# Labbeti/conette-audio-captioning

Hardware: AMD Instinct MI355X
Metric: clips_per_sec (higher is better)
Workload: dtype bf16; 1 GPU; B=64/GPU x 10 s @ 32 kHz clips, ConvNeXt encoder + beam-3 KV-cached decode (min 3 / max 20 tokens, V=5631), synthetic seeded checkpoint; batch_per_gpu=64, global_batch=64, beam_size=3, parallelism=dp1, world_size_observed=1, allreduce_of_ones=1, decode_group=2, decode_streams=2, encode_streams=1, input_batches_rotated=4

## Files before the change

### conette-audio-captioning_amd/csrc/encoder.hip

```cpp
#include <stddef.h>

#include "ctx.h"
#include <type_traits>
#include <utility>

__device__ int g_cn_nonfinite;
__device__ __forceinline__ void cn_watch_stat(float v) {
  if (!(__builtin_fabsf(v) <= 3.0e38f)) atomicAdd(&g_cn_nonfinite, 1);
}

#include "gemm2.h"
#include "mlp_rc2.h"
#include "mlp_rs16.h"
#include "mlp_sp.h"
#include "down_fused.h"

template <typename XT>
__global__ __launch_bounds__(256) void cn_stem_mfma_kernel(const float* __restrict__ in, int F, int H0, long n_pos,
                                                           const float* __restrict__ w , const float* __restrict__ bias,
                                                           const float* __restrict__ ln_w, const float* __restrict__ ln_b,
                                                           XT* __restrict__ out) {
  __shared__ __attribute__((aligned(16))) float s_p[3 * 96];
  for (int i = threadIdx.x; i < 3 * 96; i += 256) s_p[i] = i < 96 ? bias[i] : i < 192 ? ln_w[i - 96] : ln_b[i - 192];
  const int lane = threadIdx.x & 63, j = lane & 31, h = lane >> 5;
  float a[3][8];
#pragma unroll
  for (int t = 0; t < 3; ++t)
#pragma unroll
    for (int s = 0; s < 8; ++s) a[t][s] = w[(4 * (s >> 1) + 2 * h + (s & 1)) * 96 + 32 * t + cn_rc2_chan(j)];
  __syncthreads();
  const long n_tiles = (n_pos + 31) >> 5;
  const long n_waves = (long)gridDim.x * 4;
  for (long tile = (long)blockIdx.x * 4 + (threadIdx.x >> 6); tile < n_tiles; tile += n_waves) {
    const long pos = tile * 32 + j;
    const long p = pos < n_pos ? pos : n_pos - 1;
    const int wq = (int)(p % 56);
    const long tt = p / 56;
    const int hh = (int)(tt % H0);
    const int b = (int)(tt / H0);
    f32x2 xv[4];
#pragma unroll
    for (int i = 0; i < 4; ++i) {
      const int r = 4 * hh - 4 + i;
      xv[i] = f32x2{0.f, 0.f};
      if (r >= 0 && r < F) xv[i] = *(const f32x2*)(in + ((size_t)b * F + r) * CN_N_MELS + 4 * wq + 2 * h);
    }
    f32x16 acc[3];
#pragma unroll
    for (int t = 0; t < 3; ++t)
#pragma unroll
      for (int u = 0; u < 2; ++u) {
        const f32x4 b0 = *(const f32x4*)(s_p + 32 * t + 16 * u + 8 * h), b1 = *(const f32x4*)(s_p + 32 * t + 16 * u + 8 * h + 4);
#pragma unroll
        for (int e = 0; e < 4; ++e) acc[t][8 * u + e] = b0[e], acc[t][8 * u + 4 + e] = b1[e];
      }
#pragma unroll
    for (int s = 0; s < 8; ++s)
#pragma unroll
      for (int t = 0; t < 3; ++t) acc[t] = __builtin_amdgcn_mfma_f32_32x32x2f32(a[t][s], xv[s >> 1][s & 1], acc[t], 0, 0, 0);
    float sum = 0.f;
#pragma unroll
    for (int t = 0; t < 3; ++t)
#pragma unroll
      for (int r = 0; r < 16; ++r) sum += acc[t][r];
    sum += __shfl_xor(sum, 32);
    const float mean = sum * (1.0f / 96.0f);
    float v2 = 0.f;
#pragma unroll
    for (int t = 0; t < 3; ++t)
#pragma unroll
      for (int r = 0; r < 16; ++r) {
        acc[t][r] -= mean;
        v2 = fmaf(acc[t][r], acc[t][r], v2);
      }
    v2 += __shfl_xor(v2, 32);
    const float rstd = 1.0f / sqrtf(v2 * (1.0f / 96.0f) + 1e-6f);
    if (pos < n_pos) {
      XT* o = out + (size_t)pos * 96 + 8 * h;
#pragma unroll
      for (int t = 0; t < 3; ++t)
#pragma unroll
        for (int u = 0; u < 2; ++u) {
          const int ch = 32 * t + 16 * u + 8 * h;
          float v[8];
#pragma unroll
          for (int q = 0; q < 2; ++q) {
            const f32x4 lw = *(const f32x4*)(s_p + 96 + ch + 4 * q), lb = *(const f32x4*)(s_p + 192 + ch + 4 * q);
#pragma unroll
            for (int e = 0; e < 4; ++e) v[4 * q + e] = acc[t][8 * u + 4 * q + e] * rstd * lw[e] + lb[e];
          }
          if constexpr (sizeof(XT) == 2) {
            *(cn_h8<XT>*)(o + 32 * t + 16 * u) = cn_h8<XT>{cn_from_f32<XT>(v[0]), cn_from_f32<XT>(v[1]), cn_from_f32<XT>(v[2]), cn_from_f32<XT>(v[3]),
                                                          cn_from_f32<XT>(v[4]), cn_from_f32<XT>(v[5]), cn_from_f32<XT>(v[6]), cn_from_f32<XT>(v[7])};
          } else {
            *(f32x4*)(o + 32 * t + 16 * u) = f32x4{v[0], v[1], v[2], v[3]};
            *(f32x4*)(o + 32 * t + 16 * u + 4) = f32x4{v[4], v[5], v[6], v[7]};
          }
        }
    }
  }
}

__device__ unsigned long long g_dw_prof[8];
#define DW_STAMP(i)                                                   \
  if (dbg) {                                                          \
    const unsigned long long t_ = clock64();                          \
    if ((threadIdx.x & 63) == 0) atomicAdd(&g_dw_prof[i], t_ - t_prev); \
    t_prev = t_;                                                      \
  }

template <int C, int S, int TH> struct DwTile {
  static constexpr int NCHUNK = C / 4;
  static constexpr int PITCH4 = NCHUNK | 1;
  static constexpr int PITCH = PITCH4 * 4;
};

template <int... U, typename F> __device__ __forceinline__ void cn_static_for(std::integer_sequence<int, U...>, F&& f) {
  (f(std::integral_constant<int, U>{}), ...);
}
__device__ __forceinline__ void cn_dw_pin1(float& v) { asm volatile("" : "+v"(v) : : "memory"); }
template <int TH, size_t... I> __device__ __forceinline__ void cn_dw_pin(float (&acc)[TH][4], std::index_sequence<I...>) {
  (cn_dw_pin1(acc[I / 4][I % 4]), ...);
}
__device__ __forceinline__ void cn_dw_opaque(unsigned& v) { asm volatile("" : "+v"(v)); }

template <typename T, typename XT, int C, int S, int TH, bool CLAMPED = false>
__global__ __launch_bounds__((C > 384 ? 384 : C) * S) void cn_dwconv_ln_kernel(const XT* __restrict__ x, int H, int W, int tiles_h,
                                                            int tiles_w, const float* __restrict__ dw_w ,
                                                            const unsigned* __restrict__ dw_wp ,
                                                            const float* __restrict__ dw_b,
                                                            const float* __restrict__ ln_w,
                                                            const float* __restrict__ ln_b, T* __restrict__ y,
                                                            int dbg) {
  extern __shared__ __attribute__((aligned(16))) char smem_raw[];
  float* s_v = (float*)smem_raw;
  unsigned long long t_prev = dbg ? clock64() : 0;
  constexpr int NP = TH * 4;
  constexpr int CT = C > 384 ? 384 : C;
  constexpr int PITCH = DwTile<C, S, TH>::PITCH;
  const int tid = threadIdx.x;
  const int c0 = tid % CT, sidx = tid / CT;
  int bid = cn_xcd_remap(blockIdx.x, gridDim.x);
  const int tw = bid % tiles_w;
  bid /= tiles_w;
  const int th = bid % tiles_h;
  const int b = bid / tiles_h;
  const int h0 = th * TH, w0 = tw * (4 * S) + sidx * 4;

  int wcl[10];
  bool wok[10];
#pragma unroll
  for (int q = 0; q < 10; ++q) {
    const int ww = w0 - 3 + q;
    wok[q] = (ww >= 0) && (ww < W);
    wcl[q] = min(max(ww, 0), W - 1) * C;
  }
#pragma unroll 1
  for (int c = c0; c < C; c += CT) {
  float acc[TH][4];
  const float bias = dw_b[c];
#pragma unroll
  for (int a = 0; a < TH; ++a)
#pragma unroll
    for (int e = 0; e < 4; ++e) acc[a][e] = bias;
  const XT* xb = x + (size_t)b * H * W * C + c;
  const bool interior = (h0 >= 3) && (h0 + TH + 3 <= H) && (w0 >= 3) && (w0 + 4 + 3 <= W);
  if constexpr (sizeof(XT) == 2) {
    static_assert(TH % 2 == 0, "row pairs");
    cn_h2 ke[3][7], ko[3][7];
#pragma unroll
    for (int a = 0; a < 3; ++a)
#pragma unroll
      for (int j = 0; j < 7; ++j) {
        ke[a][j] = __builtin_bit_cast(cn_h2, dw_wp[(a * 7 + j) * C + c]);
        ko[a][j] = __builtin_bit_cast(cn_h2, dw_wp[(21 + a * 7 + j) * C + c]);
      }
    DW_STAMP(0)
    auto fma_pair = [&](int r, const cn_h2 (&p)[10]) {
#pragma unroll
      for (int oh = 0; oh < TH; ++oh) {
        const int i = r - oh;
        if (i < -1 || i > 6) continue;
#pragma unroll
        for (int q = 0; q < 10; ++q)
#pragma unroll
          for (int ow = 0; ow < 4; ++ow) {
            const int j = q - ow;
            if (j < 0 || j > 6) continue;
            if (i == -1) acc[oh][ow] = fmaf((float)p[q][1], (float)ke[0][j][0], acc[oh][ow]);
            else if (i == 6) acc[oh][ow] = fmaf((float)p[q][0], (float)ko[2][j][1], acc[oh][ow]);
            else if ((i & 1) == 0) acc[oh][ow] = __builtin_amdgcn_fdot2(p[q], ke[i >> 1][j], acc[oh][ow], false);
            else acc[oh][ow] = __builtin_amdgcn_fdot2(p[q], ko[i >> 1][j], acc[oh][ow], false);
          }
      }
    };
    constexpr int NPR = (TH + 6) / 2;
    if constexpr (!CLAMPED) {
      const bool left = (w0 == 0), right = (w0 + 7 > W);
      const unsigned oL = 2u * (unsigned)((left ? 0 : w0 - 3) * C + c), oM = 2u * (unsigned)(w0 * C + c);
      const unsigned oR = 2u * (unsigned)((right ? w0 + 1 : w0 + 4) * C + c);
      constexpr unsigned SEL_PAIR = 0x05040100u, SEL_ZERO = 0x0c0c0c0cu;
      const unsigned selL = left ? SEL_ZERO : SEL_PAIR, selR = right ? SEL_ZERO : SEL_PAIR;
      const char* xc = (const char*)(x + (size_t)b * H * W * C);
      const bool rows_in = (h0 >= 3) && (h0 + TH + 3 <= H);
      const unsigned rows = ((1u << min(TH + 6, H + 3 - h0)) - 1u) & ~((1u << max(0, 3 - h0)) - 1u);
      auto conv = [&](auto check_rows) {
        constexpr bool CHECK = decltype(check_rows)::value;
        auto load_row = [&](int r, unsigned (&v)[10]) {
          const int hh = h0 - 3 + r;
          if (!CHECK || ((rows >> r) & 1u)) {
            const char* xr = xc + (size_t)hh * W * C * 2;
#pragma unroll
            for (int q = 0; q < 10; ++q)
              v[q] = *(const unsigned short*)(q < 3 ? xr + (size_t)oL + q * C * 2 : q < 7 ? xr + (size_t)oM + (q - 3) * C * 2 : xr + (size_t)oR + (q - 7) * C * 2);
          } else {
#pragma unroll
            for (int q = 0; q < 10; ++q) v[q] = 0u;
          }
        };
        auto pack = [&](const unsigned (&v0)[10], const unsigned (&v1)[10], cn_h2 (&p)[10]) {
#pragma unroll
          for (int q = 0; q < 10; ++q)
            p[q] = __builtin_bit_cast(cn_h2, __builtin_amdgcn_perm(v1[q], v0[q], q < 3 ? selL : q < 7 ? SEL_PAIR : selR));
        };
        auto pin = [&]() {
          if constexpr (CHECK) cn_dw_pin(acc, std::make_index_sequence<TH * 4>{});
        };
        unsigned a0[10], a1[10], b0[10], b1[10];
        cn_h2 p[10];
        load_row(0, a0);
        load_row(1, a1);
        cn_static_for(std::make_integer_sequence<int, (NPR + 1) / 2>{}, [&](auto k) {
          constexpr int u = 2 * decltype(k)::value;
          if (u + 1 < NPR) {
            load_row(2 * u + 2, b0);
            load_row(2 * u + 3, b1);
          }
          pack(a0, a1, p);
          fma_pair(2 * u, p);
          pin();
          if (u + 2 < NPR) {
            load_row(2 * u + 4, a0);
            load_row(2 * u + 5, a1);
          }
          if (u + 1 < NPR) {
            pack(b0, b1, p);
            fma_pair(2 * (u + 1), p);
            pin();
          }
        });
      };
      if (rows_in) conv(std::false_type{});
      else conv(std::true_type{});
    } else {
#pragma unroll
      for (int u = 0; u < NPR; ++u) {
        const int hh0 = h0 - 3 + 2 * u, hh1 = hh0 + 1;
        const bool ok0 = (hh0 >= 0) && (hh0 < H), ok1 = (hh1 >= 0) && (hh1 < H);
        const XT* x0 = xb + (size_t)min(max(hh0, 0), H - 1) * W * C;
        const XT* x1 = xb + (size_t)min(max(hh1, 0), H - 1) * W * C;
        XT v0[10], v1[10];
#pragma unroll
        for (int q = 0; q < 10; ++q) v0[q] = x0[wcl[q]], v1[q] = x1[wcl[q]];
        cn_h2 p[10];
#pragma unroll
        for (int q = 0; q < 10; ++q) p[q] = cn_h2{(ok0 && wok[q]) ? v0[q] : (XT)0.f, (ok1 && wok[q]) ? v1[q] : (XT)0.f};
        fma_pair(2 * u, p);
      }
    }
  } else {
  float k[49];
#pragma unroll
  for (int i = 0; i < 49; ++i) k[i] = dw_w[i * C + c];
  DW_STAMP(0)
  auto fma_row = [&](int r, const XT (&v)[10]) {
#pragma unroll
    for (int oh = 0; oh < TH; ++oh) {
      const int i = r - oh;
      if (i < 0 || i > 6) continue;
#pragma unroll
      for (int q = 0; q < 10; ++q)
#pragma unroll
        for (int ow = 0; ow < 4; ++ow) {
          const int j = q - ow;
          if (j < 0 || j > 6) continue;
          acc[oh][ow] = fmaf((float)v[q], k[i * 7 + j], acc[oh][ow]);
        }
    }
  };
  if (interior) {
    const XT* base = xb + ((size_t)(h0 - 3) * W + (w0 - 3)) * C;
    XT va[10], vb[10];
#pragma unroll
    for (int q = 0; q < 10; ++q) va[q] = base[q * C];
#pragma unroll
    for (int r = 0; r < TH + 6; r += 2) {
      if (r + 1 < TH + 6) {
        const XT* xr = base + (size_t)(r + 1) * W * C;
#pragma unroll
        for (int q = 0; q < 10; ++q) vb[q] = xr[q * C];
      }
      fma_row(r, va);
      if (r + 2 < TH + 6) {
        const XT* xr = base + (size_t)(r + 2) * W * C;
#pragma unroll
        for (int q = 0; q < 10; ++q) va[q] = xr[q * C];
      }
      if (r + 1 < TH + 6) fma_row(r + 1, vb);
    }
  } else {
#pragma unroll
    for (int r = 0; r < TH + 6; ++r) {
      const int hh = h0 - 3 + r;
      const bool hok = (hh >= 0) && (hh < H);
      const XT* xr = xb + (size_t)min(max(hh, 0), H - 1) * W * C;
      XT v[10];
#pragma unroll
      for (int q = 0; q < 10; ++q) v[q] = xr[wcl[q]];
#pragma unroll
      for (int q = 0; q < 10; ++q) v[q] = (hok && wok[q]) ? v[q] : (XT)0.f;
      fma_row(r, v);
    }
  }
  }
#pragma unroll
  for (int oh = 0; oh < TH; ++oh)
#pragma unroll
    for (int ow = 0; ow < 4; ++ow) s_v[((sidx * NP) + oh * 4 + ow) * PITCH + c] = acc[oh][ow];
  DW_STAMP(1)
  }
  __syncthreads();
  DW_STAMP(2)

  constexpr int NPOS = NP * S, NT = CT * S, PARTS = NT / NPOS, NCHUNK = C / 4, CPT = NCHUNK / PARTS;
  static_assert(NT % NPOS == 0 && NCHUNK % PARTS == 0, "LayerNorm thread mapping");
  float* s_ps = s_v + NPOS * PITCH;
  float* s_mean = s_ps + NPOS * PARTS;
  float* s_rstd = s_mean + NPOS;
  {
    const int pos = tid % NPOS, part = tid / NPOS;
    const float* row = s_v + pos * PITCH + part * 4;
    f32x4 seg[CPT];
    float sum = 0.f;
#pragma unroll
    for (int i = 0; i < CPT; ++i) {
      seg[i] = *(const f32x4*)(row + i * PARTS * 4);
      sum += (seg[i][0] + seg[i][1]) + (seg[i][2] + seg[i][3]);
    }
    s_ps[part * NPOS + pos] = sum;
    __syncthreads();
    float mean = 0.f;
#pragma unroll
    for (int j = 0; j < PARTS; ++j) mean += s_ps[j * NPOS + pos];
    mean *= (1.0f / C);
    float sq = 0.f;
#pragma unroll
    for (int i = 0; i < CPT; ++i)
#pragma unroll
      for (int e = 0; e < 4; ++e) {
        const float d = seg[i][e] - mean;
        sq = fmaf(d, d, sq);
      }
    __syncthreads();
    s_ps[part * NPOS + pos] = sq;
    __syncthreads();
    if (part == 0) {
      float var = 0.f;
#pragma unroll
      for (int j = 0; j < PARTS; ++j) var += s_ps[j * NPOS + pos];
      s_mean[pos] = mean;
      s_rstd[pos] = 1.0f / sqrtf(var * (1.0f / C) + 1e-6f);
      cn_watch_stat(var);
    }
    __syncthreads();
  }
  DW_STAMP(3)
  constexpr int C8 = C / 8;
  static_assert(NT % C8 == 0, "a thread keeps its 8 channels over all its items: the LN affine is loaded once");
  const int c8 = (tid % C8) * 8;
  const f32x4 lw0 = *(const f32x4*)(ln_w + c8), lw1 = *(const f32x4*)(ln_w + c8 + 4);
  const f32x4 lb0 = *(const f32x4*)(ln_b + c8), lb1 = *(const f32x4*)(ln_b + c8 + 4);
  for (int item = tid; item < NPOS * C8; item += NT) {
    const int pos = item / C8;
    const int ps = pos / NP, oh = (pos % NP) >> 2, ow = pos & 3;
    const int h = h0 + oh, w = tw * (4 * S) + ps * 4 + ow;
    if (h >= H || w >= W) continue;
    const float mean = s_mean[pos], rstd = s_rstd[pos];
    const f32x4 v0 = *(const f32x4*)(s_v + pos * PITCH + c8), v1 = *(const f32x4*)(s_v + pos * PITCH + c8 + 4);
    T* dst = y + (((size_t)b * H + h) * W + w) * C + c8;
    float o[8];
#pragma unroll
    for (int i = 0; i < 8; ++i) o[i] = ((i < 4 ? v0[i] : v1[i - 4]) - mean) * rstd * (i < 4 ? lw0[i] : lw1[i - 4]) + (i < 4 ? lb0[i] : lb1[i - 4]);
    cn_store8(dst, o);
  }
  DW_STAMP(4)
}

extern "C" int conette_debug_g2prof(unsigned long long* out16, int reset) {
  if (out16) CN_HIP(hipMemcpyFromSymbol(out16, HIP_SYMBOL(g_g2_prof), 128));
  if (reset) {
    unsigned long long z[16] = {0};
    CN_HIP(hipMemcpyToSymbol(HIP_SYMBOL(g_g2_prof), z, 128));
  }
  return CN_OK;
}

extern "C" int conette_debug_dwprof(unsigned long long* out8, int reset) {
  if (out8) CN_HIP(hipMemcpyFromSymbol(out8, HIP_SYMBOL(g_dw_prof), 64));
  if (reset) {
    unsigned long long z[8] = {0, 0, 0, 0, 0, 0, 0, 0};
    CN_HIP(hipMemcpyToSymbol(HIP_SYMBOL(g_dw_prof), z, 64));
  }
  return CN_OK;
}

template <typename T, typename XT, int C, int S, int TH, bool CLAMPED>
static int launch_dwconv_as(const XT* x, int B, int H, int W, const CnBlockW& bw, T* y, hipStream_t s) {
  const int tiles_h = cn_cdiv(H, TH), tiles_w = cn_cdiv(W, 4 * S);
  constexpr int NPOS_ = TH * 4 * S, NT_ = (C > 384 ? 384 : C) * S;
  const size_t smem = ((size_t)NPOS_ * DwTile<C, S, TH>::PITCH + NPOS_ * (NT_ / NPOS_) + 2 * NPOS_) * sizeof(float);
  CN_TRY(cn_configure_lds((const void*)cn_dwconv_ln_kernel<T, XT, C, S, TH, CLAMPED>, (int)smem));
  hipLaunchKernelGGL((cn_dwconv_ln_kernel<T, XT, C, S, TH, CLAMPED>), dim3((unsigned)(B * tiles_h * tiles_w)),
                     dim3((C > 384 ? 384 : C) * S), smem, s, x, H, W, tiles_h, tiles_w, bw.dw_w, bw.dw_wp, bw.dw_b, bw.ln_w, bw.ln_b, y,
#ifdef CN_G2_PROF
                     getenv("CN_DW_DEBUG") ? atoi(getenv("CN_DW_DEBUG")) : 0);
#else
                     0);
#endif
  CN_LAUNCH_CHECK();
  return CN_OK;
}

template <typename T, typename XT, int C, int S, int TH>
static int launch_dwconv(const XT* x, int B, int H, int W, const CnBlockW& bw, T* y, hipStream_t s) {
  if constexpr (sizeof(XT) == 2) {
    if constexpr (C <= 192)
      if (W % (4 * S) == 0 && W >= 12) return launch_dwconv_as<T, XT, C, S, TH, false>(x, B, H, W, bw, y, s);
    return launch_dwconv_as<T, XT, C, S, TH, true>(x, B, H, W, bw, y, s);
  } else {
    return launch_dwconv_as<T, XT, C, S, TH, false>(x, B, H, W, bw, y, s);
  }
}

template <int C, int WW, int TH, int OW0, int NOW, typename XT>
__device__ __forceinline__ void cn_fw_conv(const XT* __restrict__ xc , int H, int h0,
                                           const float* __restrict__ dw_w, const unsigned* __restrict__ dw_wp,
                                           const float* __restrict__ dw_b, int c, float* __restrict__ s_v, int PITCH) {
  constexpr int Q0 = OW0 - 3 < 0 ? 0 : OW0 - 3, Q1 = OW0 + NOW + 3 > WW ? WW : OW0 + NOW + 3, NQ = Q1 - Q0;
  if constexpr (sizeof(XT) == 2) {
    static_assert(TH % 2 == 0, "row pairs");
    constexpr int GRP = 4095 / (2 * C) + 1, NG = (NQ + GRP - 1) / GRP;
    static_assert((GRP - 1) * C * 2 <= 4095, "a group's last column fits the immediate");
    unsigned og[NG];
#pragma unroll
    for (int g = 0; g < NG; ++g) {
      og[g] = 2u * (unsigned)((Q0 + g * GRP) * C + c);
      cn_dw_opaque(og[g]);
    }
    constexpr unsigned SEL_PAIR = 0x05040100u;
    const char* xcb = (const char*)xc;
    const bool rows_in = (h0 >= 3) && (h0 + TH + 3 <= H);
    const unsigned rows = ((1u << min(TH + 6, H + 3 - h0)) - 1u) & ~((1u << max(0, 3 - h0)) - 1u);
    cn_h2 ke[3][7], ko[3][7];
    float acc[TH][NOW];
    constexpr int WGRP = 4095 / (4 * C) + 1;
    unsigned ow = 4u * (unsigned)c;
    cn_dw_opaque(ow);
    auto load_weights = [&]() {
#pragma unroll
      for (int t0 = 0; t0 < 42; t0 += WGRP) {
        unsigned sb = (unsigned)(t0 * C * 4);
        asm volatile("" : "+s"(sb));
        const char* wb = (const char*)dw_wp + sb;
#pragma unroll
        for (int t = t0; t < t0 + WGRP && t < 42; ++t) {
          const cn_h2 w = __builtin_bit_cast(cn_h2, *(const unsigned*)(wb + (size_t)ow + (t - t0) * C * 4));
          if (t < 21) ke[t / 7][t % 7] = w;
          else ko[(t - 21) / 7][t % 7] = w;
        }
      }
    };
    auto fma_pair = [&](int r, const cn_h2 (&p)[NQ]) {
#pragma unroll
      for (int oh = 0; oh < TH; ++oh) {
        const int i = r - oh;
        if (i < -1 || i > 6) continue;
#pragma unroll
        for (int ow = 0; ow < NOW; ++ow)
#pragma unroll
          for (int j = 0; j < 7; ++j) {
            const int q = OW0 + ow + j - 3;
            if (q < 0 || q >= WW) continue;
            const cn_h2 pv = p[q - Q0];
            if (i == -1) acc[oh][ow] = fmaf((float)pv[1], (float)ke[0][j][0], acc[oh][ow]);
            else if (i == 6) acc[oh][ow] = fmaf((float)pv[0], (float)ko[2][j][1], acc[oh][ow]);
            else if ((i & 1) == 0) acc[oh][ow] = __builtin_amdgcn_fdot2(pv, ke[i >> 1][j], acc[oh][ow], false);
            else acc[oh][ow] = __builtin_amdgcn_fdot2(pv, ko[i >> 1][j], acc[oh][ow], false);
          }
      }
    };
    constexpr int NPR = (TH + 6) / 2;
    auto conv = [&](auto check_rows) {
      constexpr bool CHECK = decltype(check_rows)::value;
      auto load_row = [&](int r, unsigned (&v)[NQ]) {
        const int hh = h0 - 3 + r;
        if (!CHECK || ((rows >> r) & 1u)) {
          const char* xr = xcb + (size_t)hh * WW * C * 2;
#pragma unroll
          for (int q = 0; q < NQ; ++q) v[q] = *(const unsigned short*)(xr + (size_t)og[q / GRP] + (q % GRP) * C * 2);
        } else {
#pragma unroll
          for (int q = 0; q < NQ; ++q) v[q] = 0u;
        }
      };
      auto pack = [&](const unsigned (&v0)[NQ], const unsigned (&v1)[NQ], cn_h2 (&p)[NQ]) {
#pragma unroll
        for (int q = 0; q < NQ; ++q) p[q] = __builtin_bit_cast(cn_h2, __builtin_amdgcn_perm(v1[q], v0[q], SEL_PAIR));
      };
      auto pin = [&]() {
        if constexpr (CHECK) cn_static_for(std::make_integer_sequence<int, TH * NOW>{}, [&](auto i) { cn_dw_pin1(acc[decltype(i)::value / NOW][decltype(i)::value % NOW]); });
      };
      unsigned a0[NQ], a1[NQ], b0[NQ], b1[NQ];
      cn_h2 p[NQ];
      load_row(0, a0);
      load_row(1, a1);
      const float bias = *(const float*)((const char*)dw_b + (size_t)ow);
      load_weights();
#pragma unroll
      for (int a = 0; a < TH; ++a)
#pragma unroll
        for (int e = 0; e < NOW; ++e) acc[a][e] = bias;
      cn_static_for(std::make_integer_sequence<int, (NPR + 1) / 2>{}, [&](auto k) {
        constexpr int u = 2 * decltype(k)::value;
        if (u + 1 < NPR) {
          load_row(2 * u + 2, b0);
          load_row(2 * u + 3, b1);
        }
        pack(a0, a1, p);
        fma_pair(2 * u, p);
        pin();
        if (u + 2 < NPR) {
          load_row(2 * u + 4, a0);
          load_row(2 * u + 5, a1);
        }
        if (u + 1 < NPR) {
          pack(b0, b1, p);
          fma_pair(2 * (u + 1), p);
          pin();
        }
      });
    };
    if (rows_in) conv(std::false_type{});
    else conv(std::true_type{});
#pragma unroll
    for (int oh = 0; oh < TH; ++oh)
#pragma unroll
      for (int ow = 0; ow < NOW; ++ow) s_v[(oh * WW + OW0 + ow) * PITCH + c] = acc[oh][ow];
    return;
  }
  const XT* xb = xc + c;
  const float bias = dw_b[c];
  float k[49];
#pragma unroll
  for (int i = 0; i < 49; ++i) k[i] = dw_w[i * C + c];
  float acc[TH][NOW];
#pragma unroll
  for (int a = 0; a < TH; ++a)
#pragma unroll
    for (int e = 0; e < NOW; ++e) acc[a][e] = bias;
  auto load_row = [&](int r, XT (&v)[NQ]) {
    const int hh = h0 - 3 + r;
    if (hh >= 0 && hh < H) {
      const XT* xr = xb + (size_t)hh * WW * C;
#pragma unroll
      for (int q = 0; q < NQ; ++q) v[q] = xr[(Q0 + q) * C];
    } else {
#pragma unroll
      for (int q = 0; q < NQ; ++q) v[q] = (XT)0.f;
    }
  };
  auto fma_row = [&](int r, const XT (&v)[NQ]) {
#pragma unroll
    for (int oh = 0; oh < TH; ++oh) {
      const int i = r - oh;
      if (i < 0 || i > 6) continue;
#pragma unroll
      for (int ow = 0; ow < NOW; ++ow)
#pragma unroll
        for (int j = 0; j < 7; ++j) {
          const int q = OW0 + ow + j - 3;
          if (q < 0 || q >= WW) continue;
          acc[oh][ow] = fmaf((float)v[q - Q0], k[i * 7 + j], acc[oh][ow]);
        }
    }
  };
  XT va[NQ], vb[NQ];
  load_row(0, va);
#pragma unroll
  for (int r = 0; r < TH + 6; r += 2) {
    if (r + 1 < TH + 6) load_row(r + 1, vb);
    fma_row(r, va);
    if (r + 2 < TH + 6) load_row(r + 2, va);
    if (r + 1 < TH + 6) fma_row(r + 1, vb);
  }
#pragma unroll
  for (int oh = 0; oh < TH; ++oh)
#pragma unroll
    for (int ow = 0; ow < NOW; ++ow) s_v[(oh * WW + OW0 + ow) * PITCH + c] = acc[oh][ow];
}

template <typename T, typename XT, int C, int WW, int TH, int SPLIT>
__global__ __launch_bounds__(C* SPLIT > 384 ? 768 : 384) void cn_dwconv_ln_fw_kernel(const XT* __restrict__ x, int H, int tiles_h,
                                                              const float* __restrict__ dw_w , const unsigned* __restrict__ dw_wp,
                                                              const float* __restrict__ dw_b,
                                                              const float* __restrict__ ln_w,
                                                              const float* __restrict__ ln_b, T* __restrict__ y) {
  extern __shared__ __attribute__((aligned(16))) char smem_raw[];
  float* s_v = (float*)smem_raw;
  constexpr int CT = C * SPLIT > 384 ? 768 : 384, NPOS = TH * WW, PITCH = C + 4, NW = CT / 64;
  static_assert(SPLIT == 1 || (SPLIT == 2 && C == 384 && WW % 2 == 0), "the width is split in two only at C = 384");
  float* s_mean = s_v + NPOS * PITCH;
  float* s_rstd = s_mean + NPOS;
  const int tid = threadIdx.x, lane = tid & 63, wave = tid >> 6;
  int bid = cn_xcd_remap(blockIdx.x, gridDim.x);
  const int th = bid % tiles_h;
  const int b = bid / tiles_h;
  const int h0 = th * TH;
  const XT* xb0 = x + (size_t)b * H * WW * C;

  if constexpr (SPLIT == 1) {
#pragma unroll 1
    for (int c = tid; c < C; c += CT) cn_fw_conv<C, WW, TH, 0, WW, XT>(xb0, H, h0, dw_w, dw_wp, dw_b, c, s_v, PITCH);
  } else {
    const int c = tid < C ? tid : tid - C;
    if (tid < C)
      cn_fw_conv<C, WW, TH, 0, WW / 2, XT>(xb0, H, h0, dw_w, dw_wp, dw_b, c, s_v, PITCH);
    else
      cn_fw_conv<C, WW, TH, WW / 2, WW / 2, XT>(xb0, H, h0, dw_w, dw_wp, dw_b, c, s_v, PITCH);
  }
  __syncthreads();
  constexpr int VPL = C / 64;
  for (int p0 = wave * 2; p0 < NPOS; p0 += NW * 2) {
    const int p1 = min(p0 + 1, NPOS - 1);
    float a0[VPL], a1[VPL], s0 = 0.f, s1 = 0.f;
#pragma unroll
    for (int i = 0; i < VPL; ++i) {
      a0[i] = s_v[p0 * PITCH + i * 64 + lane];
      a1[i] = s_v[p1 * PITCH + i * 64 + lane];
      s0 += a0[i];
      s1 += a1[i];
    }
    const float m0 = cn_wave_sum_dpp(s0) * (1.0f / C), m1 = cn_wave_sum_dpp(s1) * (1.0f / C);
    float q0 = 0.f, q1 = 0.f;
#pragma unroll
    for (int i = 0; i < VPL; ++i) {
      q0 = fmaf(a0[i] - m0, a0[i] - m0, q0);
      q1 = fmaf(a1[i] - m1, a1[i] - m1, q1);
    }
    q0 = cn_wave_sum_dpp(q0);
    q1 = cn_wave_sum_dpp(q1);
    if (lane == 0) {
      s_mean[p0] = m0;
      s_rstd[p0] = 1.0f / sqrtf(q0 * (1.0f / C) + 1e-6f);
      s_mean[p1] = m1;
      s_rstd[p1] = 1.0f / sqrtf(q1 * (1.0f / C) + 1e-6f);
      cn_watch_stat(q0 + q1);
    }
  }
  __syncthreads();
  constexpr int C8 = C / 8;
  static_assert(CT % C8 == 0, "a thread keeps its 8 channels over all its items: the LN affine is loaded once");
  const int c8 = (tid % C8) * 8;
  const f32x4 lw0 = *(const f32x4*)(ln_w + c8), lw1 = *(const f32x4*)(ln_w + c8 + 4);
  const f32x4 lb0 = *(const f32x4*)(ln_b + c8), lb1 = *(const f32x4*)(ln_b + c8 + 4);
  for (int item = tid; item < NPOS * C8; item += CT) {
    const int pos = item / C8;
    const int h = h0 + pos / WW, w = pos % WW;
    if (h >= H) continue;
    const float mean = s_mean[pos], rstd = s_rstd[pos];
    const f32x4 v0 = *(const f32x4*)(s_v + pos * PITCH + c8), v1 = *(const f32x4*)(s_v + pos * PITCH + c8 + 4);
    T* dst = y + (((size_t)b * H + h) * WW + w) * C + c8;
    float o[8];
#pragma unroll
    for (int i = 0; i < 8; ++i) o[i] = ((i < 4 ? v0[i] : v1[i - 4]) - mean) * rstd * (i < 4 ? lw0[i] : lw1[i - 4]) + (i < 4 ? lb0[i] : lb1[i - 4]);
    cn_store8(dst, o);
  }
}

#ifndef CN_DW96_S
#define CN_DW96_S 2
#endif
#ifndef CN_DW96_TH
#define CN_DW96_TH 12
#endif
#ifndef CN_DW192_S
#define CN_DW192_S 1
#endif
#ifndef CN_DW192_TH
#define CN_DW192_TH 12
#endif
#ifndef CN_FW_SPLIT
#define CN_FW_SPLIT 2
#endif
#ifndef CN_FW_TH
#define CN_FW_TH 4
#endif
template <typename T, typename XT, int C, int WW, int TH, int SPLIT = 1>
static int launch_dwconv_fw(const XT* x, int B, int H, const CnBlockW& bw, T* y, hipStream_t s) {
  const int tiles_h = cn_cdiv(H, TH);
  const size_t smem = ((size_t)TH * WW * (C + 4) + 2 * TH * WW) * sizeof(float);
  CN_TRY(cn_configure_lds((const void*)cn_dwconv_ln_fw_kernel<T, XT, C, WW, TH, SPLIT>, (int)smem));
  hipLaunchKernelGGL((cn_dwconv_ln_fw_kernel<T, XT, C, WW, TH, SPLIT>), dim3((unsigned)(B * tiles_h)), dim3(C * SPLIT > 384 ? 768 : 384), smem, s, x, H,
                     tiles_h, bw.dw_w, bw.dw_wp, bw.dw_b, bw.ln_w, bw.ln_b, y);
  CN_LAUNCH_CHECK();
  return CN_OK;
}

template <typename T, typename XT, int C>
__global__ __launch_bounds__(256) void cn_ln_patchify_kernel(const XT* __restrict__ x, int H, int W, long n_pos,
                                                             const float* __restrict__ ln_w,
                                                             const float* __restrict__ ln_b, T* __restrict__ p) {
  constexpr int PER = C > 192 ? 2 : 1;
  constexpr int LANES = C / 4 / PER;
  constexpr int SLOTS = LANES <= 32 ? 2 : 1;
  constexpr int PPW = 4;
  const int lane = threadIdx.x & 63;
  const int sl = SLOTS == 2 ? lane >> 5 : 0, ll = SLOTS == 2 ? lane & 31 : lane;
  const bool act = ll < LANES;
  const long pos0 = ((long)blockIdx.x * 4 + (threadIdx.x >> 6)) * (PPW * SLOTS);
  if (pos0 >= n_pos) return;
  const int H2 = H / 2, W2 = W / 2;
  f32x4 v[PPW][PER];
#pragma unroll
  for (int u = 0; u < PPW; ++u) {
    const long pos = min(pos0 + u * SLOTS + sl, n_pos - 1);
#pragma unroll
    for (int i = 0; i < PER; ++i)
      v[u][i] = act ? cn_ld4(x + (size_t)pos * C + 4 * (ll + LANES * i)) : f32x4{0.f, 0.f, 0.f, 0.f};
  }
  f32x4 gw[PER], gb[PER];
#pragma unroll
  for (int i = 0; i < PER; ++i) {
    gw[i] = act ? *(const f32x4*)(ln_w + 4 * (ll + LANES * i)) : f32x4{0.f, 0.f, 0.f, 0.f};
    gb[i] = act ? *(const f32x4*)(ln_b + 4 * (ll + LANES * i)) : f32x4{0.f, 0.f, 0.f, 0.f};
  }
  auto group_sum = [&](float s) {
    s = cn_sum8_dpp(s);
    s += cn_dpp<0x140>(s);
    s += __shfl_xor(s, 16);
    if (SLOTS == 1) s += __shfl_xor(s, 32);
    return s;
  };
#pragma unroll
  for (int u = 0; u < PPW; ++u) {
    const long pos = pos0 + u * SLOTS + sl;
    float s = 0.f;
#pragma unroll
    for (int i = 0; i < PER; ++i) s += (v[u][i][0] + v[u][i][1]) + (v[u][i][2] + v[u][i][3]);
    const float mean = group_sum(s) * (1.0f / C);
    float s2 = 0.f;
#pragma unroll
    for (int i = 0; i < PER; ++i)
#pragma unroll
      for (int e = 0; e < 4; ++e) {
        const float d = act ? v[u][i][e] - mean : 0.f;
        s2 = fmaf(d, d, s2);
      }
    const float rstd = 1.0f / sqrtf(group_sum(s2) * (1.0f / C) + 1e-6f);
    if (pos >= n_pos || !act) continue;
    if (ll == 0) cn_watch_stat(rstd);
    const int w = (int)(pos % W);
    const long t = pos / W;
    const int h = (int)(t % H);
    const int b = (int)(t / H);
    if (h >= 2 * H2 || w >= 2 * W2) continue;
    T* o = p + ((((size_t)b * H2 + (h >> 1)) * W2 + (w >> 1)) * 4 + ((h & 1) * 2 + (w & 1))) * C;
#pragma unroll
    for (int i = 0; i < PER; ++i) {
      const int cc = 4 * (ll + LANES * i);
      cn_store4(o + cc, (v[u][i][0] - mean) * rstd * gw[i][0] + gb[i][0], (v[u][i][1] - mean) * rstd * gw[i][1] + gb[i][1],
                (v[u][i][2] - mean) * rstd * gw[i][2] + gb[i][2], (v[u][i][3] - mean) * rstd * gw[i][3] + gb[i][3]);
    }
  }
}

template <typename T, typename XT>
__global__ __launch_bounds__(256) void cn_frame_mean_kernel(const XT* __restrict__ x, int W, int C,
                                                            float* __restrict__ fe, T* __restrict__ fe_t) {
  const size_t bt = blockIdx.x;
  bool bad = false;
  for (int c = threadIdx.x; c < C; c += 256) {
    float s = 0.f;
    for (int w = 0; w < W; ++w) s += cn_ld1(x + (bt * W + w) * C + c);
    const float m = s / (float)W;
    bad |= !(__builtin_fabsf(m) <= 3.0e38f);
    fe[bt * C + c] = m;
    if (fe_t) fe_t[bt * C + c] = cn_from_f32<T>(m);
  }
  if (__syncthreads_or(bad ? 1 : 0) && threadIdx.x == 0) atomicAdd(&g_cn_nonfinite, 1);
}

template <typename T>
__global__ __launch_bounds__(256) void cn_clip_pool_ln_kernel(const float* __restrict__ fe, int Tn,
                                                              const float* __restrict__ ln_w,
                                                              const float* __restrict__ ln_b, T* __restrict__ out) {
  __shared__ float s_red[8];
  const int b = blockIdx.x, tid = threadIdx.x;
  float v[3];
  float s = 0.f;
#pragma unroll
  for (int i = 0; i < 3; ++i) {
    const int c = tid + 256 * i;
    float mx = -INFINITY, sm = 0.f;
    const float* col = fe + (size_t)b * Tn * CN_FEAT + c;
    int t = 0;
    for (; t + 8 <= Tn; t += 8) {
      float a[8];
#pragma unroll
      for (int u = 0; u < 8; ++u) a[u] = col[(size_t)(t + u) * CN_FEAT];
#pragma unroll
      for (int u = 0; u < 8; ++u) {
        mx = fmaxf(mx, a[u]);
        sm += a[u];
      }
    }
    for (; t < Tn; ++t) {
      const float a = col[(size_t)t * CN_FEAT];
      mx = fmaxf(mx, a);
      sm += a;
    }
    v[i] = mx + sm / (float)Tn;
    s += v[i];
  }
  s = cn_wave_sum(s);
  if ((tid & 63) == 0) s_red[tid >> 6] = s;
  __syncthreads();
  const float mean = (s_red[0] + s_red[1] + s_red[2] + s_red[3]) * (1.0f / CN_FEAT);
  float s2 = 0.f;
#pragma unroll
  for (int i = 0; i < 3; ++i) {
    const float d = v[i] - mean;
    s2 = fmaf(d, d, s2);
  }
  s2 = cn_wave_sum(s2);
  if ((tid & 63) == 0) s_red[4 + (tid >> 6)] = s2;
  __syncthreads();
  const float rstd = 1.0f / sqrtf((s_red[4] + s_red[5] + s_red[6] + s_red[7]) * (1.0f / CN_FEAT) + 1e-6f);
#pragma unroll
  for (int i = 0; i < 3; ++i) {
    const int c = tid + 256 * i;
    out[(size_t)b * CN_FEAT + c] = cn_from_f32<T>((v[i] - mean) * rstd * ln_w[c] + ln_b[c]);
  }
}

#ifndef CN_SP_NW96
#define CN_SP_NW96 12
#define CN_SP_NST96 4
#endif

struct EncGeom {
  int F, H[4], W[4];
};
static EncGeom enc_geom(int L) {
  EncGeom g;
  g.F = L / CN_HOP + 1;
  g.H[0] = (g.F + 8 - 4) / 4 + 1;
  g.W[0] = 56;
  for (int i = 1; i < 4; ++i) {
    g.H[i] = g.H[i - 1] / 2;
    g.W[i] = g.W[i - 1] / 2;
  }
  return g;
}

extern "C" int32_t conette_num_frames(int32_t n_samples) { return n_samples / CN_HOP + 1; }
extern "C" int32_t conette_num_audio_frames(int32_t n_samples) { return enc_geom(n_samples).H[3]; }

struct EncWs {
  float* logmel;
  void* x;
  void* y;
  void* h;
  void* fe_t;
  void* clip_t;
  size_t total;
};
static EncWs enc_ws(const conette_ctx* ctx, int B, int L, char* base) {
  const EncGeom g = enc_geom(L);
  const size_t es = ctx->esize;
  const size_t n0 = (size_t)B * g.H[0] * g.W[0] * 96;
  EncWs w;
  size_t off = 0;
  auto take = [&](size_t bytes) {
    char* p = base ? base + off : nullptr;
    off += cn_align(bytes);
    return p;
  };
  w.logmel = (float*)take((size_t)B * g.F * CN_N_MELS * 4);
  w.x = take((n0 + 32 * 96) * 4);
  w.y = take((n0 + 32 * 96) * es);
  w.h = take(n0 * 4 * es);
  w.fe_t = take((size_t)B * g.H[3] * CN_FEAT * es);
  w.clip_t = take((size_t)B * CN_FEAT * es);
  w.total = off;
  return w;
}

extern "C" size_t conette_encode_workspace_bytes(const conette_ctx* ctx, int32_t batch, int32_t n_samples) {
  return enc_ws(ctx, batch, n_samples, nullptr).total;
}

template <typename T, typename XT>
static int dwconv_dispatch(int C, const XT* x, int B, int H, int W, const CnBlockW& bw, T* y, hipStream_t s) {
  switch (C) {
    case 96: return launch_dwconv<T, XT, 96, CN_DW96_S, sizeof(XT) == 2 ? CN_DW96_TH : 8>(x, B, H, W, bw, y, s);
    case 192: return launch_dwconv<T, XT, 192, CN_DW192_S, sizeof(XT) == 2 ? CN_DW192_TH : 8>(x, B, H, W, bw, y, s);
    case 384:
      if (W == 14) return launch_dwconv_fw<T, XT, 384, 14, CN_FW_TH, CN_FW_SPLIT>(x, B, H, bw, y, s);
      return launch_dwconv<T, XT, 384, 1, 4>(x, B, H, W, bw, y, s);
    case 768:
      if (W == 7) return launch_dwconv_fw<T, XT, 768, 7, 4>(x, B, H, bw, y, s);
      return launch_dwconv<T, XT, 768, 1, 4>(x, B, H, W, bw, y, s);
  }
  cn_set_error("dwconv: unsupported C=%d", C);
  return CN_ERR_ARG;
}

static int tap_copy(float* dst, const float* src, size_t n, hipStream_t s) {
  if (dst) CN_HIP(hipMemcpyAsync(dst, src, n * sizeof(float), hipMemcpyDeviceToDevice, s));
  return CN_OK;
}
static __global__ void cn_tap_widen_kernel(const half_t* __restrict__ src, float* __restrict__ dst, size_t n) {
  for (size_t i = (size_t)blockIdx.x * blockDim.x + threadIdx.x; i < n; i += (size_t)gridDim.x * blockDim.x) dst[i] = (float)src[i];
}
static int tap_copy(float* dst, const half_t* src, size_t n, hipStream_t s) {
  if (dst) {
    hipLaunchKernelGGL(cn_tap_widen_kernel, dim3((unsigned)((n + 255) / 256 < 4096 ? (n + 255) / 256 : 4096)), dim3(256), 0, s, src, dst, n);
    CN_LAUNCH_CHECK();
  }
  return CN_OK;
}

template <typename T, typename XT>
static int encode_impl(conette_ctx* ctx, const float* wave, int B, int L, float* frame_embs, float* clip_probs,
                       const conette_encode_taps* taps, char* wsp, hipStream_t s) {
  const EncGeom g = enc_geom(L);
  EncWs ws = enc_ws(ctx, B, L, wsp);
  T* y = (T*)ws.y;
  T* hbuf = (T*)ws.h;
  XT* const wsx = (XT*)ws.x;
  {
    CnProfScope ps(ctx, CONETTE_PROF_FRONTEND, s);
    CN_TRY(cn_frontend(ctx, wave, B, L, ws.logmel, s));
  }
  if (taps) CN_TRY(tap_copy(taps->logmel, ws.logmel, (size_t)B * g.F * CN_N_MELS, s));
  {
    const long n_pos = (long)B * g.H[0] * g.W[0];
    CnProfScope ps(ctx, CONETTE_PROF_STEM, s);
    const long n_tiles = (n_pos + 31) / 32;
    const unsigned grid = (unsigned)std::min<long>((n_tiles + 3) / 4, 8L * ctx->n_cu);
    hipLaunchKernelGGL((cn_stem_mfma_kernel<XT>), dim3(grid), dim3(256), 0, s, ws.logmel, g.F, g.H[0], n_pos, ctx->stem_w, ctx->stem_b,
                       ctx->stem_ln_w, ctx->stem_ln_b, wsx);
    CN_LAUNCH_CHECK();
    if (taps) CN_TRY(tap_copy(taps->stem, wsx, (size_t)n_pos * 96, s));
  }
  XT* xc = wsx;
  int blk = 0;
  for (int st = 0; st < 4; ++st) {
    const int C = CN_DIMS[st], H = g.H[st], W = g.W[st];
    const long P = (long)B * H * W;
    if (st > 0) {
      const int Cp = CN_DIMS[st - 1], Hp = g.H[st - 1], Wp = g.W[st - 1];
      const long n_in = (long)B * Hp * Wp;
      const CnDownW& dw = ctx->down[st - 1];
      CnProfScope ps(ctx, CONETTE_PROF_DOWNSAMPLE, s);
      bool fused_down = false;
      if constexpr (CnIsH16<T>::value) if (Cp <= 192 && dw.fused != nullptr) {
        XT* xo = xc == wsx ? (XT*)ws.h : wsx;
        const int nb = ctx->n_cu - ctx->enc_reserved_cus;
        if (Cp == 96) CN_TRY((cn_launch_down_fused<96, 8, T, XT>(xc, B, Hp, Wp, dw.fused, xo, nb, s)));
        else CN_TRY((cn_launch_down_fused_ring<192, 4, 4, 3, T, XT>(xc, B, Hp, Wp, dw.fused, xo, nb, s)));
        xc = xo;
        if (taps) CN_TRY(tap_copy(taps->down[st], xc, (size_t)P * C, s));
        fused_down = true;
      }
      if (!fused_down) {
      const int ppb = Cp == 96 ? 32 : 16;
      const dim3 pg((unsigned)((n_in + ppb - 1) / ppb));
// ... 143 lines not shown
```

Baseline: 13560 clips/s.

## Restructure dwconv LayerNorm epilogues: batched loads, fewer barriers, unrolled constant-offset stores

Reworks the LayerNorm epilogue of both depthwise-conv kernels. Variance partials now go to a separate LDS buffer, which removes one barrier, and the LN affine loads are hoisted above the barrier. The output loop is fully unrolled with all LDS reads issued up front and stores placed at compile-time offsets. The full-width kernel computes per-position statistics for several positions at once with interleaved DPP and shuffle reductions, and the debug clock stamps are compiled out for most instantiations. This adds LDS use and register pressure in exchange for more memory-level parallelism and less index arithmetic.

```diff
diff --git a/conette-audio-captioning_amd/csrc/encoder.hip b/conette-audio-captioning_amd/csrc/encoder.hip
--- a/conette-audio-captioning_amd/csrc/encoder.hip
+++ b/conette-audio-captioning_amd/csrc/encoder.hip
@@ -102,11 +102,18 @@
 }
 
 __device__ unsigned long long g_dw_prof[8];
-#define DW_STAMP(i)                                                   \
-  if (dbg) {                                                          \
-    const unsigned long long t_ = clock64();                          \
-    if ((threadIdx.x & 63) == 0) atomicAdd(&g_dw_prof[i], t_ - t_prev); \
-    t_prev = t_;                                                      \
+#ifdef CN_G2_PROF
+#define DW_STAMPS_ALWAYS true
+#else
+#define DW_STAMPS_ALWAYS false
+#endif
+#define DW_STAMP(i)                                                     \
+  if constexpr (DW_STAMPS_ALWAYS || C > 384) {                          \
+    if (dbg) {                                                          \
+      const unsigned long long t_ = clock64();                          \
+      if ((threadIdx.x & 63) == 0) atomicAdd(&g_dw_prof[i], t_ - t_prev); \
+      t_prev = t_;                                                      \
+    }                                                                   \
   }
 
 template <int C, int S, int TH> struct DwTile {
@@ -123,6 +130,13 @@
   (cn_dw_pin1(acc[I / 4][I % 4]), ...);
 }
 __device__ __forceinline__ void cn_dw_opaque(unsigned& v) { asm volatile("" : "+v"(v)); }
+__device__ __forceinline__ void cn_dw_opaque_s(unsigned& v) { asm volatile("" : "+s"(v)); }
+__device__ __forceinline__ void cn_dw_pin_item(float& mean, float& rstd, f32x4& v0, f32x4& v1) {
+  asm volatile("" : "+v"(mean), "+v"(rstd), "+v"(v0), "+v"(v1) : : "memory");
+}
+__device__ __forceinline__ void cn_dw_pin_affine(f32x4& lw0, f32x4& lw1, f32x4& lb0, f32x4& lb1) {
+  asm volatile("" : "+v"(lw0), "+v"(lw1), "+v"(lb0), "+v"(lb1));
+}
 
 template <typename T, typename XT, int C, int S, int TH, bool CLAMPED = false>
 __global__ __launch_bounds__((C > 384 ? 384 : C) * S) void cn_dwconv_ln_kernel(const XT* __restrict__ x, int H, int W, int tiles_h,
@@ -134,7 +148,7 @@
                                                             int dbg) {
   extern __shared__ __attribute__((aligned(16))) char smem_raw[];
   float* s_v = (float*)smem_raw;
-  unsigned long long t_prev = dbg ? clock64() : 0;
+  [[maybe_unused]] unsigned long long t_prev = ((DW_STAMPS_ALWAYS || C > 384) && dbg) ? clock64() : 0;
   constexpr int NP = TH * 4;
   constexpr int CT = C > 384 ? 384 : C;
   constexpr int PITCH = DwTile<C, S, TH>::PITCH;
@@ -329,14 +343,20 @@
     for (int ow = 0; ow < 4; ++ow) s_v[((sidx * NP) + oh * 4 + ow) * PITCH + c] = acc[oh][ow];
   DW_STAMP(1)
   }
+  constexpr int NPOS = NP * S, NT = CT * S, PARTS = NT / NPOS, NCHUNK = C / 4, CPT = NCHUNK / PARTS;
+  static_assert(NT % NPOS == 0 && NCHUNK % PARTS == 0, "LayerNorm thread mapping");
+  constexpr int C8 = C / 8, PSTEP = NT / C8, NI = NPOS / PSTEP;
+  static_assert(NT % C8 == 0, "a thread keeps its 8 channels over all its items: the LN affine is loaded once");
+  static_assert(PSTEP % 4 == 0 && NP % PSTEP == 0 && NPOS % PSTEP == 0, "an item step moves whole rows of a patch: (h, w) advance by constants");
+  float* s_ps = s_v + NPOS * PITCH;
+  float* s_pq = s_ps + NPOS * PARTS;
+  float* s_mean = s_pq + NPOS * PARTS;
+  float* s_rstd = s_mean + NPOS;
+  const int c8 = (tid % C8) * 8, pb = tid / C8;
+  f32x4 lw0 = *(const f32x4*)(ln_w + c8), lw1 = *(const f32x4*)(ln_w + c8 + 4);
+  f32x4 lb0 = *(const f32x4*)(ln_b + c8), lb1 = *(const f32x4*)(ln_b + c8 + 4);
   __syncthreads();
   DW_STAMP(2)
-
-  constexpr int NPOS = NP * S, NT = CT * S, PARTS = NT / NPOS, NCHUNK = C / 4, CPT = NCHUNK / PARTS;
-  static_assert(NT % NPOS == 0 && NCHUNK % PARTS == 0, "LayerNorm thread mapping");
-  float* s_ps = s_v + NPOS * PITCH;
-  float* s_mean = s_ps + NPOS * PARTS;
-  float* s_rstd = s_mean + NPOS;
   {
     const int pos = tid % NPOS, part = tid / NPOS;
     const float* row = s_v + pos * PITCH + part * 4;
@@ -361,13 +381,12 @@
         const float d = seg[i][e] - mean;
         sq = fmaf(d, d, sq);
       }
-    __syncthreads();
-    s_ps[part * NPOS + pos] = sq;
+    s_pq[part * NPOS + pos] = sq;
     __syncthreads();
     if (part == 0) {
       float var = 0.f;
 #pragma unroll
-      for (int j = 0; j < PARTS; ++j) var += s_ps[j * NPOS + pos];
+      for (int j = 0; j < PARTS; ++j) var += s_pq[j * NPOS + pos];
       s_mean[pos] = mean;
       s_rstd[pos] = 1.0f / sqrtf(var * (1.0f / C) + 1e-6f);
       cn_watch_stat(var);
@@ -375,23 +394,36 @@
     __syncthreads();
   }
   DW_STAMP(3)
-  constexpr int C8 = C / 8;
-  static_assert(NT % C8 == 0, "a thread keeps its 8 channels over all its items: the LN affine is loaded once");
-  const int c8 = (tid % C8) * 8;
-  const f32x4 lw0 = *(const f32x4*)(ln_w + c8), lw1 = *(const f32x4*)(ln_w + c8 + 4);
-  const f32x4 lb0 = *(const f32x4*)(ln_b + c8), lb1 = *(const f32x4*)(ln_b + c8 + 4);
-  for (int item = tid; item < NPOS * C8; item += NT) {
-    const int pos = item / C8;
-    const int ps = pos / NP, oh = (pos % NP) >> 2, ow = pos & 3;
-    const int h = h0 + oh, w = tw * (4 * S) + ps * 4 + ow;
-    if (h >= H || w >= W) continue;
-    const float mean = s_mean[pos], rstd = s_rstd[pos];
-    const f32x4 v0 = *(const f32x4*)(s_v + pos * PITCH + c8), v1 = *(const f32x4*)(s_v + pos * PITCH + c8 + 4);
-    T* dst = y + (((size_t)b * H + h) * W + w) * C + c8;
-    float o[8];
-#pragma unroll
-    for (int i = 0; i < 8; ++i) o[i] = ((i < 4 ? v0[i] : v1[i - 4]) - mean) * rstd * (i < 4 ? lw0[i] : lw1[i - 4]) + (i < 4 ? lb0[i] : lb1[i - 4]);
-    cn_store8(dst, o);
+  {
+    const int ohb = pb >> 2, owb = pb & 3;
+    const int hlim = H - h0 - ohb, wlim = W - tw * (4 * S) - owb;
+    unsigned off = (unsigned)sizeof(T) * (unsigned)((ohb * W + owb) * C + c8);
+    cn_dw_opaque(off);
+    char* yb = (char*)(y + (((size_t)b * H + h0) * W + tw * (4 * S)) * C);
+    const float* sv = s_v + pb * PITCH + c8;
+    float mean[NI], rstd[NI];
+    f32x4 v0[NI], v1[NI];
+#pragma unroll
+    for (int k = 0; k < NI; ++k) {
+      mean[k] = s_mean[pb + k * PSTEP];
+      rstd[k] = s_rstd[pb + k * PSTEP];
+      v0[k] = *(const f32x4*)(sv + k * PSTEP * PITCH);
+      v1[k] = *(const f32x4*)(sv + k * PSTEP * PITCH + 4);
+    }
+#pragma unroll
+    for (int k = 0; k < NI; ++k) cn_dw_pin_item(mean[k], rstd[k], v0[k], v1[k]);
+    cn_dw_pin_affine(lw0, lw1, lb0, lb1);
+    cn_static_for(std::make_integer_sequence<int, NI>{}, [&](auto kk) {
+      constexpr int k = decltype(kk)::value, DH = (k * PSTEP % NP) / 4, DW = (k * PSTEP / NP) * 4;
+      if (DH < hlim && DW < wlim) {
+        T* dst = (T*)(yb + ((size_t)DH * W + DW) * C * sizeof(T) + (size_t)off);
+        float o[8];
+#pragma unroll
+        for (int i = 0; i < 8; ++i)
+          o[i] = ((i < 4 ? v0[k][i] : v1[k][i - 4]) - mean[k]) * rstd[k] * (i < 4 ? lw0[i] : lw1[i - 4]) + (i < 4 ? lb0[i] : lb1[i - 4]);
+        cn_store8(dst, o);
+      }
+    });
   }
   DW_STAMP(4)
 }
@@ -418,7 +450,7 @@
 static int launch_dwconv_as(const XT* x, int B, int H, int W, const CnBlockW& bw, T* y, hipStream_t s) {
   const int tiles_h = cn_cdiv(H, TH), tiles_w = cn_cdiv(W, 4 * S);
   constexpr int NPOS_ = TH * 4 * S, NT_ = (C > 384 ? 384 : C) * S;
-  const size_t smem = ((size_t)NPOS_ * DwTile<C, S, TH>::PITCH + NPOS_ * (NT_ / NPOS_) + 2 * NPOS_) * sizeof(float);
+  const size_t smem = ((size_t)NPOS_ * DwTile<C, S, TH>::PITCH + 2 * NPOS_ * (NT_ / NPOS_) + 2 * NPOS_) * sizeof(float);
   CN_TRY(cn_configure_lds((const void*)cn_dwconv_ln_kernel<T, XT, C, S, TH, CLAMPED>, (int)smem));
   hipLaunchKernelGGL((cn_dwconv_ln_kernel<T, XT, C, S, TH, CLAMPED>), dim3((unsigned)(B * tiles_h * tiles_w)),
                      dim3((C > 384 ? 384 : C) * S), smem, s, x, H, W, tiles_h, tiles_w, bw.dw_w, bw.dw_wp, bw.dw_b, bw.ln_w, bw.ln_b, y,
@@ -638,52 +670,101 @@
     else
       cn_fw_conv<C, WW, TH, WW / 2, WW / 2, XT>(xb0, H, h0, dw_w, dw_wp, dw_b, c, s_v, PITCH);
   }
+  constexpr int C8 = C / 8, PSTEP = CT / C8, NI = (NPOS + PSTEP - 1) / PSTEP;
+  static_assert(CT % C8 == 0, "a thread keeps its 8 channels over all its items: the LN affine is loaded once");
+  const int c8 = (tid % C8) * 8, pb = tid / C8;
+  f32x4 lw0 = *(const f32x4*)(ln_w + c8), lw1 = *(const f32x4*)(ln_w + c8 + 4);
+  f32x4 lb0 = *(const f32x4*)(ln_b + c8), lb1 = *(const f32x4*)(ln_b + c8 + 4);
   __syncthreads();
-  constexpr int VPL = C / 64;
-  for (int p0 = wave * 2; p0 < NPOS; p0 += NW * 2) {
-    const int p1 = min(p0 + 1, NPOS - 1);
-    float a0[VPL], a1[VPL], s0 = 0.f, s1 = 0.f;
-#pragma unroll
-    for (int i = 0; i < VPL; ++i) {
-      a0[i] = s_v[p0 * PITCH + i * 64 + lane];
-      a1[i] = s_v[p1 * PITCH + i * 64 + lane];
-      s0 += a0[i];
-      s1 += a1[i];
-    }
-    const float m0 = cn_wave_sum_dpp(s0) * (1.0f / C), m1 = cn_wave_sum_dpp(s1) * (1.0f / C);
-    float q0 = 0.f, q1 = 0.f;
-#pragma unroll
-    for (int i = 0; i < VPL; ++i) {
-      q0 = fmaf(a0[i] - m0, a0[i] - m0, q0);
-      q1 = fmaf(a1[i] - m1, a1[i] - m1, q1);
-    }
-    q0 = cn_wave_sum_dpp(q0);
-    q1 = cn_wave_sum_dpp(q1);
-    if (lane == 0) {
-      s_mean[p0] = m0;
-      s_rstd[p0] = 1.0f / sqrtf(q0 * (1.0f / C) + 1e-6f);
-      s_mean[p1] = m1;
-      s_rstd[p1] = 1.0f / sqrtf(q1 * (1.0f / C) + 1e-6f);
-      cn_watch_stat(q0 + q1);
+  {
+    constexpr int VPL = C / 64, NPP = (NPOS + NW - 1) / NW;
+    static_assert(NPP <= 64, "a lane per position of the wave");
+    float a[NPP][VPL], sm[NPP], q[NPP];
+#pragma unroll
+    for (int j = 0; j < NPP; ++j) {
+      const int p = min(wave + j * NW, NPOS - 1);
+#pragma unroll
+      for (int i = 0; i < VPL; ++i) a[j][i] = s_v[p * PITCH + i * 64 + lane];
+    }
+    auto wave_sums = [&](float (&v)[NPP]) {
+#pragma unroll
+      for (int j = 0; j < NPP; ++j) v[j] += cn_dpp<0xB1>(v[j]);
+#pragma unroll
+      for (int j = 0; j < NPP; ++j) v[j] += cn_dpp<0x4E>(v[j]);
+#pragma unroll
+      for (int j = 0; j < NPP; ++j) v[j] += cn_dpp<0x141>(v[j]);
+#pragma unroll
+      for (int j = 0; j < NPP; ++j) v[j] += cn_dpp<0x140>(v[j]);
+      float t[NPP];
+#pragma unroll
+      for (int j = 0; j < NPP; ++j) t[j] = __shfl_xor(v[j], 16);
+#pragma unroll
+      for (int j = 0; j < NPP; ++j) v[j] += t[j];
+#pragma unroll
+      for (int j = 0; j < NPP; ++j) t[j] = __shfl_xor(v[j], 32);
+#pragma unroll
+      for (int j = 0; j < NPP; ++j) v[j] += t[j];
+    };
+#pragma unroll
+    for (int j = 0; j < NPP; ++j) {
+      sm[j] = 0.f;
+#pragma unroll
+      for (int i = 0; i < VPL; ++i) sm[j] += a[j][i];
+    }
+    wave_sums(sm);
+#pragma unroll
+    for (int j = 0; j < NPP; ++j) {
+      sm[j] *= (1.0f / C);
+      q[j] = 0.f;
+#pragma unroll
+      for (int i = 0; i < VPL; ++i) q[j] = fmaf(a[j][i] - sm[j], a[j][i] - sm[j], q[j]);
+    }
+    wave_sums(q);
+    float mj = sm[0], qj = q[0];
+#pragma unroll
+    for (int j = 1; j < NPP; ++j) {
+      mj = lane == j ? sm[j] : mj;
+      qj = lane == j ? q[j] : qj;
+    }
+    if (lane < NPP && wave + lane * NW < NPOS) {
+      const int p = wave + lane * NW;
+      s_mean[p] = mj;
+      s_rstd[p] = 1.0f / sqrtf(qj * (1.0f / C) + 1e-6f);
+      cn_watch_stat(qj);
     }
   }
   __syncthreads();
-  constexpr int C8 = C / 8;
-  static_assert(CT % C8 == 0, "a thread keeps its 8 channels over all its items: the LN affine is loaded once");
-  const int c8 = (tid % C8) * 8;
-  const f32x4 lw0 = *(const f32x4*)(ln_w + c8), lw1 = *(const f32x4*)(ln_w + c8 + 4);
-  const f32x4 lb0 = *(const f32x4*)(ln_b + c8), lb1 = *(const f32x4*)(ln_b + c8 + 4);
-  for (int item = tid; item < NPOS * C8; item += CT) {
-    const int pos = item / C8;
-    const int h = h0 + pos / WW, w = pos % WW;
-    if (h >= H) continue;
-    const float mean = s_mean[pos], rstd = s_rstd[pos];
-    const f32x4 v0 = *(const f32x4*)(s_v + pos * PITCH + c8), v1 = *(const f32x4*)(s_v + pos * PITCH + c8 + 4);
-    T* dst = y + (((size_t)b * H + h) * WW + w) * C + c8;
-    float o[8];
-#pragma unroll
-    for (int i = 0; i < 8; ++i) o[i] = ((i < 4 ? v0[i] : v1[i - 4]) - mean) * rstd * (i < 4 ? lw0[i] : lw1[i - 4]) + (i < 4 ? lb0[i] : lb1[i - 4]);
-    cn_store8(dst, o);
+  {
+    const int lim = min(NPOS, (H - h0) * WW) - pb;
+    unsigned off = (unsigned)sizeof(T) * (unsigned)(pb * C + c8);
+    cn_dw_opaque(off);
+    char* yb = (char*)(y + ((size_t)b * H + h0) * WW * C);
+    float mean[NI], rstd[NI];
+    f32x4 v0[NI], v1[NI];
+#pragma unroll
+    for (int k = 0; k < NI; ++k) {
+      const int p = (k + 1) * PSTEP > NPOS ? min(pb + k * PSTEP, NPOS - 1) : pb + k * PSTEP;
+      mean[k] = s_mean[p];
+      rstd[k] = s_rstd[p];
+      v0[k] = *(const f32x4*)(s_v + p * PITCH + c8);
+      v1[k] = *(const f32x4*)(s_v + p * PITCH + c8 + 4);
+    }
+#pragma unroll
+    for (int k = 0; k < NI; ++k) cn_dw_pin_item(mean[k], rstd[k], v0[k], v1[k]);
+    cn_dw_pin_affine(lw0, lw1, lb0, lb1);
+    cn_static_for(std::make_integer_sequence<int, NI>{}, [&](auto kk) {
+      constexpr int k = decltype(kk)::value;
+      if (k * PSTEP < lim) {
+        unsigned sk = (unsigned)(k * PSTEP * C * sizeof(T));
+        cn_dw_opaque_s(sk);
+        T* dst = (T*)(yb + (size_t)sk + (size_t)off);
+        float o[8];
+#pragma unroll
+        for (int i = 0; i < 8; ++i)
+          o[i] = ((i < 4 ? v0[k][i] : v1[k][i - 4]) - mean[k]) * rstd[k] * (i < 4 ? lw0[i] : lw1[i - 4]) + (i < 4 ? lb0[i] : lb1[i - 4]);
+        cn_store8(dst, o);
+      }
+    });
   }
 }
 
```

Result: no change. 13690 clips/s, median of 6 (+1.0%).
